# sortmerna/sortmerna

Measured on NVIDIA H100. Metric: reads/sec (150 bp vs SILVA-8), higher is better.
Workload: dtype int16x2 (DPX) / u8

## Files before the change

### sortmerna_b200/csrc/smr_levbits.h

```cpp
#pragma once
#include <cstdint>
#if defined(__CUDACC__)
#define SMR_HD __host__ __device__ __forceinline__
#else
#define SMR_HD inline
#endif

namespace smr {

SMR_HD uint32_t lb_popc(uint32_t x) {
#if defined(__CUDA_ARCH__)
  return (uint32_t)__popc(x);
#else
  return (uint32_t)__builtin_popcount(x);
#endif
}
SMR_HD int32_t lb_ctz(uint32_t x) {
#if defined(__CUDA_ARCH__)
  return __ffs((int)x) - 1;
#else
  return __builtin_ctz(x);
#endif
}
SMR_HD int32_t lb_clz(uint32_t x) {
#if defined(__CUDA_ARCH__)
  return __clz((int)x);
#else
  return __builtin_clz(x);
#endif
}

SMR_HD uint32_t neq2(uint32_t x) { return (x | (x >> 1)) & 0x55555555u; }
SMR_HD uint32_t mk2(uint32_t k) { return ((1u << (2 * k)) - 1u) & 0x55555555u; }
SMR_HD int32_t firstmis(uint32_t m, int32_t dflt) { return m ? (lb_ctz(m) >> 1) : dflt; }
SMR_HD int32_t lastmis(uint32_t m) { return m ? ((31 - lb_clz(m)) >> 1) : -1; }

SMR_HD uint32_t classify_bits(uint32_t P, uint32_t T, uint32_t pw) {
  const uint32_t A = neq2(T ^ P), B = neq2(T ^ (P >> 2)), C = neq2((T >> 2) ^ P);
  const uint32_t A9 = A & mk2(pw), A8 = A & mk2(pw - 1), B8 = B & mk2(pw - 1), C9 = C & mk2(pw);
  const bool acc7 = lastmis(B8) < firstmis(A8, (int32_t)pw - 1);
  const bool acc8 = lb_popc(A9) <= 1;
  const bool acc9 = lastmis(C9) < firstmis(A9, (int32_t)pw);
  return (acc7 ? 1u : (acc8 ? 2u : (acc9 ? 3u : 0u))) | (A9 == 0 ? 4u : 0u);
}
struct LevMasks { uint32_t m9, m8, s9, s8; };
SMR_HD LevMasks lev_masks(uint32_t pw) { return LevMasks{mk2(pw), mk2(pw - 1), 1u << (2 * pw), 1u << (2 * (pw - 1))}; }
SMR_HD bool within_one_edit(uint32_t P, uint32_t T, const LevMasks& k) {
  const uint32_t x = T ^ P, y = T ^ (P >> 2), z = (T >> 2) ^ P;
  const uint32_t A9 = (x | (x >> 1)) & k.m9, B8 = (y | (y >> 1)) & k.m8, C9 = (z | (z >> 1)) & k.m9;
  const uint32_t a8 = (A9 & k.m8) | k.s8, a9 = A9 | k.s9;
  return ((A9 & (A9 - 1u)) == 0u) | (B8 < (a8 & (0u - a8))) | (C9 < (a9 & (0u - a9)));
}
SMR_HD bool viable_bits(uint32_t P, uint32_t T, uint32_t k) {
  const uint32_t Ak = neq2(T ^ P) & mk2(k);
  if (lb_popc(Ak) <= 1) return true;
  const int32_t a = firstmis(Ak, (int32_t)k);
  if (lastmis(neq2(T ^ (P >> 2)) & mk2(k)) < a) return true;
  return lastmis(neq2((T >> 2) ^ P) & mk2(k - 1)) < a;
}

}
```

### sortmerna_b200/csrc/smr_seed.cuh

```cuda
#pragma once
#include "smr_dev.cuh"
#include "smr_levbits.h"

namespace smr {

__device__ __forceinline__ uint32_t rev_chars(uint32_t v, uint32_t pw) {
  uint32_t x = __brev(v) >> (32 - 2 * pw);
  return ((x & 0x55555555u) << 1) | ((x >> 1) & 0x55555555u);
}

__device__ __forceinline__ uint64_t window_fwd(const uint32_t* __restrict__ pk, uint32_t p, uint32_t L) {
  const uint32_t wi = p >> 4, s = 2 * (p & 15);
  const uint64_t hi = ((uint64_t)__ldg(pk + wi) << 32) | __ldg(pk + wi + 1);
  const uint64_t lo = (uint64_t)__ldg(pk + wi + 2) << 32;
  const uint64_t v = s ? ((hi << s) | (lo >> (64 - s))) : hi;
  return v >> (64 - 2 * L);
}
__device__ __forceinline__ uint64_t revcomp_bits(uint64_t v, uint32_t L) {
  uint64_t x = __brevll(v) >> (64 - 2 * L);
  x = ((x & 0x5555555555555555ull) << 1) | ((x >> 1) & 0x5555555555555555ull);
  return ~x & ((1ull << (2 * L)) - 1);
}

constexpr uint32_t kLaneSmemIds = 8;
struct LaneHits {
  uint32_t* sbuf; uint32_t* buf; uint32_t stride, cap, n; bool overflow;
};
__device__ __forceinline__ uint32_t lh_get(const LaneHits& lh, uint32_t k) { return k < kLaneSmemIds ? lh.sbuf[k * 32] : lh.buf[k * lh.stride]; }
__device__ __forceinline__ void lh_set(LaneHits& lh, uint32_t k, uint32_t id) { if (k < kLaneSmemIds) lh.sbuf[k * 32] = id; else lh.buf[k * lh.stride] = id; }

struct SeedStats { uint32_t entries, lists; };

__device__ __forceinline__ bool apply_entry(uint32_t code, uint32_t id, bool full_search, LaneHits& lh) {
  const uint32_t d1 = code & 3u;
  if (d1 == 0) return false;
  const bool z = (code & 4u) && !full_search;
  if (d1 == 2 && z) { lh.n = 1; lh_set(lh, 0, id); lh.overflow = false; return true; }
  for (uint32_t f = 0; f < lh.n && f < lh.cap; ++f) if (lh_get(lh, f) == id) return false;
  if (lh.n < lh.cap) lh_set(lh, lh.n, id); else lh.overflow = true;
  lh.n++;
  if (d1 == 1 && z) { lh.n = 1; lh_set(lh, 0, id); lh.overflow = false; return true; }
  return false;
}

__device__ __forceinline__ uint32_t pass_class(uint32_t p, uint32_t s0, uint32_t s1, uint32_t s2) {
  if (p % s0 == 0) return 0;
  if (p % s1 == 0) return 1;
  if (p % s2 == 0) return 2;
  return 3;
}

constexpr int kAccStep = 256;
constexpr int kAccCap = 384;

struct CoopSmem {
  uint4 tab[64];
  uint32_t id[kAccCap];
  uint32_t text[kAccCap];
  uint8_t meta[kAccCap];
  uint8_t own[64];
  uint16_t run[2][2][32];
  uint32_t ids[kLaneSmemIds][32];
};

template <bool INSTR>
__device__ void coop_stream(const DevIndex& ix, CoopSmem& sm, const uint32_t offF, const uint32_t cntF, const uint32_t PF,
                            const uint32_t offR, const uint32_t cntR, const uint32_t PR, const bool full_search,
                            LaneHits& lh, bool& zero, SeedStats& st) {
  const unsigned lane = lane_id();
  const uint32_t pw = ix.partialwin;
  const LevMasks km = lev_masks(pw);
  const uint4* __restrict__ ft4 = reinterpret_cast<const uint4*>(ix.ftext);
  const uint32_t gF = offF >> 3, nF = cntF ? ((offF + cntF + 7u) >> 3) - gF : 0u;
  const uint32_t gR = offR >> 3, nR = cntR ? ((offR + cntR + 7u) >> 3) - gR : 0u;
  const uint32_t inF = warp_incl_scan_u32(nF), inR = warp_incl_scan_u32(nR);
  const uint32_t totF = __shfl_sync(kFull, inF, 31), E = totF + __shfl_sync(kFull, inR, 31);
  const uint32_t exF = nF ? inF - nF : kNoneDev, exR = nR ? totF + inR - nR : kNoneDev;
  if (INSTR) { st.entries += cntF + cntR; st.lists += (cntF ? 1u : 0u) + (cntR ? 1u : 0u); }
  if (E == 0) return;
  const uint32_t lt = (1u << lane) - 1u, le = lt | (1u << lane);
  {
    const unsigned mF = __ballot_sync(kFull, nF != 0), mR = __ballot_sync(kFull, nR != 0);
    if (nF) { const uint32_t k = __popc(mF & lt); sm.tab[k] = make_uint4(gF - exF, PF, offF, offF + cntF); sm.own[k] = (uint8_t)lane; }
    if (nR) { const uint32_t k = __popc(mF) + __popc(mR & lt); sm.tab[k] = make_uint4(gR - exR, PR, offR, offR + cntR); sm.own[k] = (uint8_t)(lane | 32u); }
  }
  __syncwarp();
  uint32_t cum = 0, nacc = 0;
  uint32_t kn, gn, Pn; uint4 q0n, q1n;
  auto fetch = [&](const uint32_t e0) {
    const uint32_t dF = exF - e0, dR = exR - e0;
    const uint32_t bit = (dF < 32u ? (1u << dF) : 0u) | (dR < 32u ? (1u << dR) : 0u);
    const uint32_t starts = __reduce_or_sync(kFull, bit);
    const uint32_t e = e0 + lane;
    kn = cum + __popc(starts & le) - 1u;
    cum += __popc(starts);
    const uint2 t = *reinterpret_cast<const uint2*>(&sm.tab[kn]);
    gn = t.x + e; Pn = t.y;
    q0n = make_uint4(0, 0, 0, 0); q1n = q0n;
    if (e < E) { q0n = __ldg(ft4 + 2 * (size_t)gn); q1n = __ldg(ft4 + 2 * (size_t)gn + 1); }
  };
  fetch(0);
  for (uint32_t e0 = 0; e0 < E; e0 += 32) {
    const uint32_t k = kn, g = gn, P = Pn; const uint4 q0 = q0n, q1 = q1n;
    if (e0 + 32 < E) fetch(e0 + 32);
    const uint32_t hit8 = (within_one_edit(P, q0.x, km) ? 1u : 0u) | (within_one_edit(P, q0.y, km) ? 2u : 0u) |
                          (within_one_edit(P, q0.z, km) ? 4u : 0u) | (within_one_edit(P, q0.w, km) ? 8u : 0u) |
                          (within_one_edit(P, q1.x, km) ? 16u : 0u) | (within_one_edit(P, q1.y, km) ? 32u : 0u) |
                          (within_one_edit(P, q1.z, km) ? 64u : 0u) | (within_one_edit(P, q1.w, km) ? 128u : 0u);
    const bool any = e0 + lane < E && hit8;
    const unsigned am = __ballot_sync(kFull, any);
    if (am) {
      uint32_t mk = 0;
      const uint32_t i0 = 8u * g;
      if (any) {
        const uint2 t = *reinterpret_cast<const uint2*>(&sm.tab[k].z);
        const uint32_t lo = t.x > i0 ? min(t.x - i0, 8u) : 0u, hi = min(t.y - i0, 8u);
        mk = hit8 & ((1u << hi) - 1u) & ~((1u << lo) - 1u);
      }
      const uint32_t nm = __popc(mk);
      const unsigned b0 = __ballot_sync(kFull, nm & 1u), b1 = __ballot_sync(kFull, nm & 2u), b2 = __ballot_sync(kFull, nm & 4u),
                     b3 = __ballot_sync(kFull, nm & 8u);
      uint32_t slot = nacc + __popc(b0 & lt) + 2u * __popc(b1 & lt) + 4u * __popc(b2 & lt) + 8u * __popc(b3 & lt);
      const uint8_t own = sm.own[k];
      while (mk) {
        const uint32_t j = (uint32_t)__ffs((int)mk) - 1u;
        mk &= mk - 1u;
        const uint4 q = j < 4 ? q0 : q1;
        const uint32_t jj = j & 3u;
        sm.text[slot] = jj == 0 ? q.x : (jj == 1 ? q.y : (jj == 2 ? q.z : q.w));
        sm.id[slot] = i0 + j;
        sm.meta[slot] = own;
        ++slot;
      }
      nacc += __popc(b0) + 2u * __popc(b1) + 4u * __popc(b2) + 8u * __popc(b3);
    }
    if (nacc && (nacc > (uint32_t)(kAccCap - kAccStep) || e0 + 32 >= E)) {
      sm.run[0][0][lane] = 0; sm.run[0][1][lane] = 0; sm.run[1][0][lane] = 0; sm.run[1][1][lane] = 0;
      __syncwarp();
      for (uint32_t i = lane; i < nacc; i += 32) {
        sm.id[i] = __ldg(ix.fid + sm.id[i]);
        const uint32_t m = sm.meta[i];
        const uint32_t prev = i ? sm.meta[i - 1] : 0xFFu, next = i + 1 < nacc ? sm.meta[i + 1] : 0xFFu;
        if (m != prev) sm.run[m >> 5][0][m & 31u] = (uint16_t)i;
        if (m != next) sm.run[m >> 5][1][m & 31u] = (uint16_t)(i + 1);
      }
      __syncwarp();
#pragma unroll
      for (int h = 0; h < 2; ++h) {
        const uint32_t end = sm.run[h][1][lane], P = h ? PR : PF;
        for (uint32_t i = sm.run[h][0][lane]; i < end && !zero; ++i)
          zero = apply_entry(classify_bits(P, sm.text[i], pw), sm.id[i], full_search, lh);
      }
      nacc = 0;
      __syncwarp();
    }
  }
  __syncwarp();
}

struct DevBatch {
  uint32_t nreads;
  const uint8_t* seq04;
  const uint32_t* seq_off;
  const uint32_t* pk03;
  const uint32_t* pk03alt;
  const uint32_t* pk_off;
  const uint8_t* has_n;
  uint32_t hit_scale;
  uint32_t seq_base0;
  uint32_t r0;
  uint2* hits;
  size_t hits_stride;
  uint32_t cnt_stride;
  uint32_t* cost;
  uint32_t* bins;
  uint32_t* bin_count;
  uint16_t* hit_db;
  uint32_t* hit_cnt;
  uint32_t* flags;
  ReadState* state;
  unsigned long long* counters;
};

__device__ __forceinline__ uint32_t hit_cap(const DevBatch& b, uint32_t r) { return b.hit_scale * (2u * (b.seq_off[r + 1] - b.seq_off[r]) + 32u); }
__device__ __forceinline__ size_t hit_base(const DevBatch& b, uint32_t part, uint32_t r) {
  return (size_t)part * b.hits_stride + (size_t)b.hit_scale * (2ull * (b.seq_off[r] - b.seq_base0) + 32ull * (r - b.r0));
}
constexpr int kCostBins = 24;

__global__ void pack_reads_kernel(DevBatch b, uint32_t* pk03, uint32_t* pk03alt, uint8_t* has_n) {
  const uint32_t warp = (blockIdx.x * blockDim.x + threadIdx.x) >> 5, nwarps = (gridDim.x * blockDim.x) >> 5;
  const unsigned lane = lane_id();
  for (uint32_t r = b.r0 + warp; r < b.r0 + b.nreads; r += nwarps) {
    const uint32_t o = b.seq_off[r], len = b.seq_off[r + 1] - o;
    const uint32_t wo = b.pk_off[r], nw = b.pk_off[r + 1] - wo;
    bool anyn = false;
    for (uint32_t w = lane; w < nw; w += 32) {
      uint32_t a = 0, t = 0;
      for (uint32_t k = 0; k < 16; ++k) {
        const uint32_t i = w * 16 + k;
        uint32_t c = i < len ? b.seq04[o + i] : 0u;
        uint32_t ca = c, ct = c;
        if (c > 3) { ca = 0; ct = 3; anyn = anyn || (i < len); }
        a |= ca << (30 - 2 * k); t |= ct << (30 - 2 * k);
      }
      pk03[wo + w] = a;
      if (pk03alt) pk03alt[wo + w] = t;
    }
    anyn = __any_sync(kFull, anyn);
    if (lane == 0) has_n[r] = anyn ? 1 : 0;
  }
}

struct SeedWin { uint4 lf, lr; uint32_t keyf, keyr, p, var; bool active; };
__device__ __forceinline__ SeedWin seed_window(const DevIndex& ix, const uint32_t* __restrict__ pk, const uint32_t* __restrict__ pka, uint32_t len,
                                               uint32_t L, uint32_t pw, uint32_t npos, uint32_t step, uint32_t s0, uint32_t s1, uint32_t s2,
                                               uint32_t v_lo, uint32_t nq, uint32_t qq) {
  SeedWin w;
  const uint32_t vr = (qq >= npos ? 1u : 0u) + (qq >= 2 * npos ? 1u : 0u);
  w.var = v_lo + vr; w.p = (qq - vr * npos) * step;
  w.active = qq < nq;
  if (w.active && step == 1) w.active = (w.p % s0 == 0) || (w.p % s1 == 0) || (w.p % s2 == 0);
  w.keyf = w.keyr = 0;
  w.lf = w.lr = make_uint4(0, 0, 0, 0);
  if (w.active) {
    uint64_t V;
    if (w.var == kVarFwd) V = window_fwd(pk, w.p, L);
    else V = revcomp_bits(window_fwd(w.var == kVarRevT ? pk : pka, len - w.p - L, L), L);
    w.keyf = (uint32_t)(V >> (2 * pw)); w.keyr = (uint32_t)(V & ((1ull << (2 * pw)) - 1));
    w.lf = __ldg(&ix.flookup[w.keyf]);
    w.lr = __ldg(&ix.flookup[w.keyr]);
  }
  return w;
}

constexpr int kSeedWarpsPerCta = 4;
#ifndef SMR_SEED_MIN_CTAS
#define SMR_SEED_MIN_CTAS 8
#endif
constexpr int kSeedCtasPerSm = SMR_SEED_MIN_CTAS;
constexpr int kSeedGrab = 4;
constexpr int kLaneHitCap = 128;

template <bool INSTR>
__global__ void __launch_bounds__(kSeedWarpsPerCta * 32, kSeedCtasPerSm)
seed_kernel(DevIndex ix, DevBatch b, DevParams prm, uint32_t* lane_hits_g, uint32_t cap_g, uint32_t* next_read) {
  __shared__ CoopSmem s_coop[kSeedWarpsPerCta];
  const unsigned lane = lane_id();
  const uint32_t wic = threadIdx.x >> 5;
  const uint32_t warp = blockIdx.x * kSeedWarpsPerCta + wic;
  const uint32_t L = ix.lnwin, pw = ix.partialwin;
  const bool full = prm.is_full_search != 0;
  CoopSmem& sm = s_coop[wic];
  LaneHits lh;
  lh.sbuf = &sm.ids[0][lane]; lh.buf = lane_hits_g + (size_t)warp * cap_g * 32 + lane; lh.stride = 32; lh.cap = cap_g;
  SeedStats st{0, 0};
  uint32_t n_windows = 0, n_short = 0;
  const bool single = (prm.is_forward != 0) != (prm.is_reverse != 0);
  const bool do_fwd = !(single && prm.is_reverse), do_rev = !(single && prm.is_forward);
  const uint32_t s0 = ix.skip[0], s1 = ix.skip[1], s2 = ix.skip[2];
  const uint32_t step = (s0 % s2 == 0 && s1 % s2 == 0) ? s2 : 1u;

  for (uint32_t g0 = 0;;) {
    if (lane == 0) g0 = atomicAdd(next_read, (uint32_t)kSeedGrab);
    g0 = __shfl_sync(kFull, g0, 0);
    if (g0 >= b.nreads) break;
  for (uint32_t r = b.r0 + g0; r < b.r0 + min(g0 + (uint32_t)kSeedGrab, b.nreads); ++r) {
    const uint32_t len = b.seq_off[r + 1] - b.seq_off[r];
    const uint32_t cnt_idx = ix.slot * b.cnt_stride + (r - b.r0);
    if (lane == 0) b.hit_cnt[cnt_idx] = 0;
    if (len < L) { n_short += (lane == 0 && ix.is_last); continue; }
    if (b.flags[r]) continue;
    const bool hasn = b.has_n[r] != 0;
    const uint32_t* pk = b.pk03 + b.pk_off[r];
    const uint32_t* pka = hasn ? b.pk03alt + b.pk_off[r] : pk;
    const uint32_t npos = (len - L) / step + 1;
    const size_t region = hit_base(b, ix.slot, r); const uint32_t region_cap = hit_cap(b, r);
    uint32_t total = 0, flags = 0, cost = 0;
    const uint32_t nvar = hasn ? 3u : 2u;
    const uint32_t v_lo = do_fwd ? 0u : 1u, v_hi = do_rev ? nvar : 1u;
    const uint32_t nq = (v_hi - v_lo) * npos;
    SeedWin nx = seed_window(ix, pk, pka, len, L, pw, npos, step, s0, s1, s2, v_lo, nq, lane);
    for (uint32_t q0 = 0; q0 < nq; q0 += 32) {
      const SeedWin w = nx;
      if (q0 + 32 < nq) nx = seed_window(ix, pk, pka, len, L, pw, npos, step, s0, s1, s2, v_lo, nq, q0 + 32 + lane);
      lh.n = 0; lh.overflow = false;
      n_windows += w.active ? 1u : 0u;
      bool zero = false;
      coop_stream<INSTR>(ix, sm, w.lf.x, w.lf.y, rev_chars(w.keyr, pw), w.lr.z, w.lr.w, w.keyf, full, lh, zero, st);
      if (lh.overflow) flags |= kOvfSeedLane;
      const uint32_t n = lh.overflow ? 0u : lh.n;
      const unsigned hm = __ballot_sync(kFull, n != 0);
      if (hm) {
        const uint32_t incl = warp_incl_scan_u32(n), tot = __shfl_sync(kFull, incl, 31);
        if (total + tot > region_cap) { flags |= kOvfSeedRegion; }
        else if (n) {
          const size_t base = region + total + incl - n;
          const uint32_t tag = w.p | (w.var << 24) | (pass_class(w.p, s0, s1, s2) << 28);
          for (uint32_t k = 0; k < n; ++k) {
            const uint32_t id = lh_get(lh, k);
            b.hits[base + k] = make_uint2(id, tag);
            cost += __ldg(ix.pos_off + id + 1) - __ldg(ix.pos_off + id);
          }
        }
        total += tot;
      }
      __syncwarp();
    }
    flags = __reduce_or_sync(kFull, flags);
    cost = warp_sum_u32(min(cost, 1u << 24));
    if (lane == 0) {
      b.hit_cnt[cnt_idx] = (flags & kOvfSeedRegion) ? 0u : total;
      if (flags) atomicOr(&b.flags[r], flags);
      if (total) atomicAdd(&b.cost[r - b.r0], max(cost, 1u));
    }
  }
  }
  const uint32_t ns = warp_sum_u32(n_short);
  if (lane == 0 && ns) atomicAdd(&b.counters[dcNumShort], (unsigned long long)ns);
  if (INSTR) {
    const uint64_t w = warp_sum_u64(n_windows), ne = warp_sum_u64(st.entries), nl = warp_sum_u64(st.lists);
    if (lane == 0) { atomicAdd(&b.counters[dcWindows], (unsigned long long)w); atomicAdd(&b.counters[dcEntries], (unsigned long long)ne); atomicAdd(&b.counters[dcBuckets], (unsigned long long)nl); }
  }
}

__global__ void bin_kernel(DevBatch b) {
  const uint32_t i = blockIdx.x * blockDim.x + threadIdx.x;
  if (i >= b.nreads) return;
  const uint32_t c = b.cost[i];
  if (c == 0 || b.flags[b.r0 + i]) return;
  const uint32_t bin = min((uint32_t)(kCostBins - 1), 31u - (uint32_t)__clz(c));
  const uint32_t slot = atomicAdd(&b.bin_count[bin], 1u);
  b.bins[(size_t)bin * b.cnt_stride + slot] = b.r0 + i;
}

__global__ void __launch_bounds__(kSeedWarpsPerCta * 32)
seed_debug_kernel(DevIndex ix, const uint8_t* seq03, const uint32_t* seq_off, const uint32_t* win_read, const uint32_t* win_pos, uint32_t nwin,
                  uint32_t* ids, uint32_t cap, uint32_t* counts, uint8_t* zero, int full_search, int mode) {
  __shared__ CoopSmem s_coop[kSeedWarpsPerCta];
  const uint32_t k = blockIdx.x * blockDim.x + threadIdx.x;
  const bool active = k < nwin;
  const uint32_t pw = ix.partialwin;
  uint64_t V = 0;
  if (active) {
    const uint8_t* sq = seq03 + seq_off[win_read[k]] + win_pos[k];
    for (uint32_t i = 0; i < ix.lnwin; ++i) V = (V << 2) | (sq[i] & 3u);
  }
  CoopSmem& sm = s_coop[threadIdx.x >> 5];
  LaneHits lh; lh.sbuf = &sm.ids[0][threadIdx.x & 31]; lh.buf = ids + (size_t)(active ? k : 0) * cap; lh.stride = 1; lh.cap = active ? cap : 0; lh.n = 0; lh.overflow = false;
  SeedStats st{0, 0};
  bool z = false;
  const bool full = full_search != 0;
  const uint32_t keyf = (uint32_t)(V >> (2 * pw)), keyr = (uint32_t)(V & ((1ull << (2 * pw)) - 1));
  const uint32_t Pf = rev_chars(keyr, pw), Pr = keyf;
  if (mode == 0) {
    const uint4 lf = active ? __ldg(&ix.flookup[keyf]) : make_uint4(0, 0, 0, 0);
    const uint4 lr = active ? __ldg(&ix.flookup[keyr]) : make_uint4(0, 0, 0, 0);
    coop_stream<false>(ix, sm, lf.x, lf.y, Pf, lr.z, lr.w, Pr, full, lh, z, st);
  } else if (active) {
    const uint4 lf = __ldg(&ix.flookup[keyf]);
    for (uint32_t i = lf.x; i < lf.x + lf.y && !z; ++i) z = apply_entry(classify_bits(Pf, __ldg(ix.ftext + i), pw), __ldg(ix.fid + i), full, lh);
    if (!z) {
      const uint4 lr = __ldg(&ix.flookup[keyr]);
      for (uint32_t i = lr.z; i < lr.z + lr.w && !z; ++i) z = apply_entry(classify_bits(Pr, __ldg(ix.ftext + i), pw), __ldg(ix.fid + i), full, lh);
    }
  }
  if (active) {
    counts[k] = lh.n; zero[k] = z ? 1 : 0;
    for (uint32_t f = 0; f < lh.n && f < lh.cap && f < kLaneSmemIds; ++f) lh.buf[f] = lh.sbuf[f * 32];
  }
}

}
```

Before: 5.628 million.

## Use cheap half-window screen then warp-parallel classify and compact candidates

Replaces the exact within-one-edit filter with a cheaper pigeonhole-style screen: a candidate passes if either half matches exactly or a shifted deletion/insertion alignment matches. Classification of accepted candidates moves out of the per-lane serial apply loop into a warp-parallel pass that compacts out non-matching entries and stores the code in place of the text. The aim is to reduce per-entry filter ALU work and per-lane serial classify divergence. The screen is looser than the exact filter, so more false candidates reach the accumulation buffer and the compaction pass adds shuffles and syncs.

```diff
diff --git a/sortmerna_b200/csrc/smr_levbits.h b/sortmerna_b200/csrc/smr_levbits.h
--- a/sortmerna_b200/csrc/smr_levbits.h
+++ b/sortmerna_b200/csrc/smr_levbits.h
@@ -51,6 +51,18 @@
   const uint32_t a8 = (A9 & k.m8) | k.s8, a9 = A9 | k.s9;
   return ((A9 & (A9 - 1u)) == 0u) | (B8 < (a8 & (0u - a8))) | (C9 < (a9 & (0u - a9)));
 }
+struct HalfMasks { uint32_t lo, hi, del, ins; };
+SMR_HD uint32_t char_bits(uint32_t a, uint32_t b) {
+  return (uint32_t)((1ull << (2 * b)) - 1ull) & ~(uint32_t)((1ull << (2 * a)) - 1ull);
+}
+SMR_HD HalfMasks half_masks(uint32_t pw) {
+  const uint32_t h = pw / 2;
+  return HalfMasks{char_bits(0, h), char_bits(h, pw), char_bits(h, pw - 1), char_bits(h + 1, pw + 1)};
+}
+SMR_HD bool half_screen(uint32_t P, uint32_t Pd, uint32_t Pi, uint32_t T, const HalfMasks& m) {
+  const uint32_t x = T ^ P;
+  return ((x & m.lo) == 0u) | ((x & m.hi) == 0u) | (((T ^ Pd) & m.del) == 0u) | (((T ^ Pi) & m.ins) == 0u);
+}
 SMR_HD bool viable_bits(uint32_t P, uint32_t T, uint32_t k) {
   const uint32_t Ak = neq2(T ^ P) & mk2(k);
   if (lb_popc(Ak) <= 1) return true;
diff --git a/sortmerna_b200/csrc/smr_seed.cuh b/sortmerna_b200/csrc/smr_seed.cuh
--- a/sortmerna_b200/csrc/smr_seed.cuh
+++ b/sortmerna_b200/csrc/smr_seed.cuh
@@ -69,7 +69,7 @@
                             LaneHits& lh, bool& zero, SeedStats& st) {
   const unsigned lane = lane_id();
   const uint32_t pw = ix.partialwin;
-  const LevMasks km = lev_masks(pw);
+  const HalfMasks km = half_masks(pw);
   const uint4* __restrict__ ft4 = reinterpret_cast<const uint4*>(ix.ftext);
   const uint32_t gF = offF >> 3, nF = cntF ? ((offF + cntF + 7u) >> 3) - gF : 0u;
   const uint32_t gR = offR >> 3, nR = cntR ? ((offR + cntR + 7u) >> 3) - gR : 0u;
@@ -85,7 +85,7 @@
     if (nR) { const uint32_t k = __popc(mF) + __popc(mR & lt); sm.tab[k] = make_uint4(gR - exR, PR, offR, offR + cntR); sm.own[k] = (uint8_t)(lane | 32u); }
   }
   __syncwarp();
-  uint32_t cum = 0, nacc = 0;
+  uint32_t cum = 0, nacc = 0, ncls = 0;
   uint32_t kn, gn, Pn; uint4 q0n, q1n;
   auto fetch = [&](const uint32_t e0) {
     const uint32_t dF = exF - e0, dR = exR - e0;
@@ -103,10 +103,11 @@
   for (uint32_t e0 = 0; e0 < E; e0 += 32) {
     const uint32_t k = kn, g = gn, P = Pn; const uint4 q0 = q0n, q1 = q1n;
     if (e0 + 32 < E) fetch(e0 + 32);
-    const uint32_t hit8 = (within_one_edit(P, q0.x, km) ? 1u : 0u) | (within_one_edit(P, q0.y, km) ? 2u : 0u) |
-                          (within_one_edit(P, q0.z, km) ? 4u : 0u) | (within_one_edit(P, q0.w, km) ? 8u : 0u) |
-                          (within_one_edit(P, q1.x, km) ? 16u : 0u) | (within_one_edit(P, q1.y, km) ? 32u : 0u) |
-                          (within_one_edit(P, q1.z, km) ? 64u : 0u) | (within_one_edit(P, q1.w, km) ? 128u : 0u);
+    const uint32_t Pd = P >> 2, Pi = P << 2;
+    const uint32_t hit8 = (half_screen(P, Pd, Pi, q0.x, km) ? 1u : 0u) | (half_screen(P, Pd, Pi, q0.y, km) ? 2u : 0u) |
+                          (half_screen(P, Pd, Pi, q0.z, km) ? 4u : 0u) | (half_screen(P, Pd, Pi, q0.w, km) ? 8u : 0u) |
+                          (half_screen(P, Pd, Pi, q1.x, km) ? 16u : 0u) | (half_screen(P, Pd, Pi, q1.y, km) ? 32u : 0u) |
+                          (half_screen(P, Pd, Pi, q1.z, km) ? 64u : 0u) | (half_screen(P, Pd, Pi, q1.w, km) ? 128u : 0u);
     const bool any = e0 + lane < E && hit8;
     const unsigned am = __ballot_sync(kFull, any);
     if (am) {
@@ -134,7 +135,28 @@
       }
       nacc += __popc(b0) + 2u * __popc(b1) + 4u * __popc(b2) + 8u * __popc(b3);
     }
-    if (nacc && (nacc > (uint32_t)(kAccCap - kAccStep) || e0 + 32 >= E)) {
+    const bool last = e0 + 32 >= E;
+    if (nacc > ncls && (nacc > (uint32_t)(kAccCap - kAccStep) || last)) {
+      __syncwarp();
+      uint32_t nm = ncls;
+      for (uint32_t b = ncls; b < nacc; b += 32) {
+        const uint32_t i = b + lane;
+        const bool in = i < nacc;
+        const uint32_t m = in ? sm.meta[i] : 0u, x = in ? sm.id[i] : 0u;
+        const uint32_t Pf = __shfl_sync(kFull, PF, m & 31u), Pr = __shfl_sync(kFull, PR, m & 31u);
+        const uint32_t code = in ? classify_bits((m & 32u) ? Pr : Pf, sm.text[i], pw) : 0u;
+        const unsigned keep = __ballot_sync(kFull, (code & 3u) != 0u);
+        __syncwarp();
+        if ((code & 3u) != 0u) {
+          const uint32_t o = nm + __popc(keep & lt);
+          sm.text[o] = code; sm.id[o] = x; sm.meta[o] = (uint8_t)m;
+        }
+        nm += __popc(keep);
+        __syncwarp();
+      }
+      nacc = ncls = nm;
+    }
+    if (nacc && (nacc > (uint32_t)(kAccCap - kAccStep) || last)) {
       sm.run[0][0][lane] = 0; sm.run[0][1][lane] = 0; sm.run[1][0][lane] = 0; sm.run[1][1][lane] = 0;
       __syncwarp();
       for (uint32_t i = lane; i < nacc; i += 32) {
@@ -147,11 +169,10 @@
       __syncwarp();
 #pragma unroll
       for (int h = 0; h < 2; ++h) {
-        const uint32_t end = sm.run[h][1][lane], P = h ? PR : PF;
-        for (uint32_t i = sm.run[h][0][lane]; i < end && !zero; ++i)
-          zero = apply_entry(classify_bits(P, sm.text[i], pw), sm.id[i], full_search, lh);
-      }
-      nacc = 0;
+        const uint32_t end = sm.run[h][1][lane];
+        for (uint32_t i = sm.run[h][0][lane]; i < end && !zero; ++i) zero = apply_entry(sm.text[i], sm.id[i], full_search, lh);
+      }
+      nacc = ncls = 0;
       __syncwarp();
     }
   }
```

Result: faster. 5.925 million, median of 6 (+5.3%).
